# vivek87799/lightweight-human-pose-estimation.pytorch

Measured on AMD Instinct MI355X. Metric: frames/sec end-to-end (net+grouping) at 368px, higher is better.
Workload: dtype f32; 1 GPU; batch=1 per GPU, 368x656 frames, 1 refinement stage(s), fp32 convs / f32+f64 post, resident normalised NCHW input -> key-points + pose entries on host; 3 frame batch(es) in flight per GPU (3 engine stream(s), each step a complete pass); global_batch=1, parallelism=dp1 (frames sharded, no data-path collective), 3 stream(s) per GPU

## Files before the change

lightweight-human-pose-estimation.pytorch_amd/csrc/capi.cpp:

```cpp
#include <algorithm>
#include <cmath>
#include <cstdio>
#include <cstdlib>
#include <cstring>
#include <map>
#include <mutex>
#include <string>
#include <vector>

#include "lwp_internal.h"
#include "lwp_owners.h"

using namespace lwp;

struct lwp_context {
    int device = 0;
    Stream stream, post_own;
    hipStream_t post_stream = nullptr;
    int dtype = LWP_F32;
    Graph g;
    Tuning tune;
    std::vector<std::string> variants;
    bool record_variants = false;
    char variant_buf[kVariantCap] = {0};
// ... 685 lines not shown
    return v;
}

static inline float* buf_at(lwp_context* h, const BufRef& r) {
    const int nb = (int)h->g.bufs.size();
    char* base = (r.buf < nb ? h->bufs[r.buf] : h->tbufs[r.buf - nb]).as<char>();
    return (float*)(base + (size_t)r.coff * (h->dtype != LWP_F32 ? 2 : 4));
}
static inline int buf_level(const lwp_context* h, int buf) {
    const int nb = (int)h->g.bufs.size();
    return buf < 0 ? 0 : buf < nb ? h->g.bufs[buf].level : h->tp.bufs[buf - nb].level;
}

static int enqueue_layer(lwp_context* h, const Layer& l, const float* d_in, int N, int H, int W, float* const* d_outs_nchw,
                         const Layer* fold = nullptr, bool* folded = nullptr) {
    const bool h16 = h->dtype != LWP_F32;
    const int f16 = h->dtype == LWP_F16;
    const float* wts = h->blob(l.w_off);
    const float* bias = h->blob(l.b_off);
    int dh, dw;
    level_dims(H, W, buf_level(h, l.dst.buf), &dh, &dw);
    float* dst = buf_at(h, l.dst);
    char* vb = h->record_variants ? h->variant_buf : nullptr;
    if (vb) vb[0] = 0;
    if (l.kind == L_STEM) {
        StemParams p{d_in, wts, bias, dst, N, H, W, dh, dw, f16, h->d_zeros.as<float>()};
        p.tune = &h->tune; p.variant = vb;
        LAUNCH(h, KC_STEM, h16 ? launch_stem_bf16(p, h->stream) : launch_stem(p, h->stream));
    } else if (l.kind == L_DWPW) {
        int sh, sw;
        level_dims(H, W, buf_level(h, l.src.buf), &sh, &sw);
        DwPwParams p;
        p.in = buf_at(h, l.src); p.in_ld = l.src.ld; p.f16 = f16;
        p.dw_w = wts; p.pw_w = h->blob(l.w2_off); p.pw_b = h->blob(l.b2_off);
        p.out = dst; p.out_ld = l.dst.ld;
        p.res = l.res.buf >= 0 ? buf_at(h, l.res) : nullptr; p.res_ld = l.res.ld;
        p.zeros = h->d_zeros.as<float>();
        p.N = N; p.Hi = sh; p.Wi = sw; p.Ho = dh; p.Wo = dw; p.C = l.cin; p.cout = l.cout;
        p.stride = l.stride; p.dil = l.dil; p.act_dw = l.act; p.act_pw = l.act2;
        p.tune = &h->tune; p.variant = vb;
        LAUNCH(h, KC_PW, h16 ? launch_dwpw_bf16(p, h->stream) : launch_dwpw(p, h->stream));
    } else if (l.kind == L_DW) {
        int sh, sw;
        level_dims(H, W, buf_level(h, l.src.buf), &sh, &sw);
        DwParams p{buf_at(h, l.src), l.src.ld, wts, bias, dst, l.dst.ld, N, sh, sw, dh, dw, l.cin, l.stride, l.dil, l.act};
        p.tune = &h->tune; p.variant = vb;
        LAUNCH(h, KC_DW, launch_dw(p, h->stream));
    } else {
        GemmParams p;
        p.in = buf_at(h, l.src); p.in_ld = l.src.ld; p.f16 = f16;
        p.w = wts; p.bias = bias;
        p.wf = h16 ? nullptr : h->blob(l.w2_off);
        p.out = dst; p.out_ld = l.dst.ld;
        p.res = l.res.buf >= 0 ? buf_at(h, l.res) : nullptr; p.res_ld = l.res.ld;
        p.out_nchw = (l.out_index >= 0 && d_outs_nchw) ? d_outs_nchw[l.out_index] : nullptr;
        p.out_nchw2 = (l.out_index2 >= 0 && d_outs_nchw) ? d_outs_nchw[l.out_index2] : nullptr;
        p.out_split = l.out_split;
        p.zeros = h->d_zeros.as<float>();
        p.N = N; p.H = dh; p.W = dw;
        p.cin_pad = l.cin_pad; p.cout = l.cout; p.cout_pad = l.cout_pad; p.ks = l.ks; p.dil = l.dil; p.act = l.act;
        p.tune = &h->tune; p.variant = vb;
        if (fold) {
            p.w2 = h->blob(fold->w_off); p.bias2 = h->blob(fold->b_off);
            p.out2 = buf_at(h, fold->dst); p.out2_ld = fold->dst.ld; p.act2 = fold->act;
            p.fused2 = folded;
        }
        LAUNCH(h, l.ks == 1 ? KC_PW : KC_C3, h16 ? launch_gemm_bf16(p, h->stream) : launch_gemm(p, h->stream));
    }
    if (vb && h->cur_layer >= 0 && h->cur_layer < (int)h->variants.size()) h->variants[h->cur_layer] = vb;
    return LWP_OK;
}

static bool heads_pair_runs(const lwp_context* h, const Layer& a, const Layer& b, int64_t M) {
    if (a.fuse != LWP_MARK_HEADS_PAIR || h->tune.fuse_heads == 0) return false;
    return h->dtype != LWP_F32 ? heads_bf16_supported(a.cin_pad, a.cout_pad, b.cout_pad) : heads_f32_supported(a.cin_pad, a.cout_pad, b.cout_pad, M, &h->tune);
}

static int enqueue_heads_pair(lwp_context* h, const Layer& a, const Layer& b, int N, int H, int W, float* const* d_outs_nchw) {
    int dh, dw;
    level_dims(H, W, buf_level(h, b.dst.buf), &dh, &dw);
    HeadsParams p;
    p.in = buf_at(h, a.src); p.in_ld = a.src.ld; p.f16 = h->dtype == LWP_F16;
    p.w0 = h->blob(a.w_off); p.b0 = h->blob(a.b_off);
    p.w1 = h->blob(b.w_off); p.b1 = h->blob(b.b_off);
    p.out = buf_at(h, b.dst); p.out_ld = b.dst.ld;
    p.out_nchw = (b.out_index >= 0 && d_outs_nchw) ? d_outs_nchw[b.out_index] : nullptr;
    p.out_nchw2 = (b.out_index2 >= 0 && d_outs_nchw) ? d_outs_nchw[b.out_index2] : nullptr;
    p.out_split = b.out_split;
    p.N = N; p.H = dh; p.W = dw; p.hidden = a.cout_pad; p.cout = b.cout;
    char* vb = h->record_variants ? h->variant_buf : nullptr;
    if (vb) vb[0] = 0;
    p.tune = &h->tune; p.variant = vb;
    LAUNCH(h, KC_PW, h->dtype != LWP_F32 ? launch_heads_bf16(p, h->stream) : launch_heads_f32(p, h->stream));
    if (vb && h->cur_layer >= 0 && h->cur_layer + 1 < (int)h->variants.size()) { h->variants[h->cur_layer] = vb; h->variants[h->cur_layer + 1] = vb; }
    return LWP_OK;
}

static int enqueue_dw_copy(lwp_context* h, const Layer& l, int buf, int N, int H, int W) {
    int sh, sw, dh, dw;
    level_dims(H, W, buf_level(h, l.src.buf), &sh, &sw);
    level_dims(H, W, buf_level(h, buf), &dh, &dw);
    DwParams p{buf_at(h, l.src), l.src.ld, h->blob(l.w_off), h->blob(l.b_off), h->tbufs[buf - (int)h->g.bufs.size()].as<float>(), l.cin,
               N, sh, sw, dh, dw, l.cin, l.stride, l.dil, l.act};
    p.tune = &h->tune;
    LAUNCH(h, KC_DW, launch_dw(p, h->stream));
    return LWP_OK;
}

static int enqueue_forward(lwp_context* h, const std::vector<Layer>& ls, int begin, int end, const float* d_in, int N, int H, int W,
                           float* const* d_outs_nchw, bool retain = false) {
    int fh, fw;
    level_dims(H, W, 3, &fh, &fw);
    const int64_t M3 = (int64_t)N * fh * fw;
    int rc = LWP_OK;
    for (int i = begin; i < end && rc == LWP_OK; ++i) {
        h->cur_layer = i;
        const bool inside = i + 1 < end;
        if (inside && heads_pair_runs(h, ls[i], ls[i + 1], M3)) {
            if (retain) rc = enqueue_layer(h, ls[i], d_in, N, H, W, nullptr);
            if (!rc) rc = enqueue_heads_pair(h, ls[i], ls[i + 1], N, H, W, d_outs_nchw);
            ++i;
            continue;
        }
        if (retain && &ls == &h->tp.layers) {
            if (h->tp.dw_copy[i] >= 0) {
                rc = enqueue_dw_copy(h, ls[i], h->tp.dw_copy[i], N, H, W);
                if (rc) break;
            }
            if (h->tp.nores_copy[i] >= 0) {
                Layer c = ls[i];
                c.res = BufRef();
                c.dst.buf = h->tp.nores_copy[i]; c.dst.coff = 0;
                c.out_index = c.out_index2 = -1;
                rc = enqueue_layer(h, c, d_in, N, H, W, nullptr);
                if (rc) break;
            }
        }
        bool folded = false;
        rc = enqueue_layer(h, ls[i], d_in, N, H, W, d_outs_nchw, inside && ls[i].fuse == LWP_MARK_FOLD_NEXT_1X1 ? &ls[i + 1] : nullptr, &folded);
        if (!rc && folded) {
            if (h->record_variants && (size_t)i + 1 < h->variants.size()) h->variants[i + 1] = h->variants[i];
            ++i;
        }
    }
    h->cur_layer = -1;
    return rc;
}
static int enqueue_network(lwp_context* h, const float* d_in, int N, int H, int W, float* const* d_outs_nchw) {
    return enqueue_forward(h, h->g.layers, 0, (int)h->g.layers.size(), d_in, N, H, W, d_outs_nchw);
}

static int check_frame_shape(lwp_context* h, int N, int H, int W) {
    if (N <= 0 || H <= 0 || W <= 0) return fail(h, LWP_ERR_ARG, "bad frame shape");
    if (H < 8 || W < 8) return fail(h, LWP_ERR_ARG, "frame too small (H, W >= 8)");
    if (!h->weights_loaded) return fail(h, LWP_ERR_STATE, "weights not loaded (call lwp_load_weights first)");
    return LWP_OK;
}

static int stage_input(lwp_context* h, const float* in, int in_mem, size_t bytes, const float** d_in) {
    if (in_mem == LWP_MEM_DEVICE) { *d_in = in; return LWP_OK; }
    HIP_TRY(h, h->d_in.ensure(bytes));
    HIP_TRY(h, hipMemcpyAsync(h->d_in.as<float>(), in, bytes, hipMemcpyHostToDevice, h->stream));
    *d_in = h->d_in.as<float>();
    return LWP_OK;
}

// ... 3495 lines not shown
```

lightweight-human-pose-estimation.pytorch_amd/csrc/lwp_internal.h:

```cpp
#pragma once
#include <hip/hip_runtime.h>
#include <stdint.h>
#include <algorithm>
#include <cstdio>
#include <string>
#include <vector>

#include "../../include/lwpose.h"

namespace lwp {

struct ParamSpec {
    std::string key;
    int64_t shape[4];
    int ndim;
    int role;
};
std::vector<ParamSpec> param_table(int nref, int C, int NH, int NP);

enum LayerKind { L_STEM = 0, L_DW = 1, L_GEMM = 2, L_DWPW = 3 };
enum Act { ACT_NONE = 0, ACT_RELU = 1, ACT_ELU = 2 };
enum KClass { KC_STEM = 0, KC_DW = 1, KC_PW = 2, KC_C3 = 3, KC_POST = 4, KC_OTHER = 5, KC_COUNT = 6 };

struct BufRef {
// ... 11 lines not shown
    int kind = L_GEMM;
    std::string name;
    std::string conv_key;
    std::string bn_key;
    bool has_bias = false;
    int cin = 0, cout = 0, ks = 1, stride = 1, dil = 1, act = ACT_NONE;
    BufRef src, dst, res;
    int out_index = -1;
    int out_index2 = -1, out_split = 0;
    std::vector<WBlock> blocks;
    int64_t macs_per_pixel = 0;
    int fuse = LWP_MARK_NONE;
    size_t w_off = 0, b_off = 0;
    int cin_pad = 0, cout_pad = 0;
    std::string conv2_key, bn2_key;
    int act2 = ACT_NONE;
    size_t w2_off = 0, b2_off = 0;
};

struct BufSpec {
    int level;
    int channels;
    bool has_pad = false;
};

struct Graph {
    int nref, C, NH, NP;
    std::vector<BufSpec> bufs;
    std::vector<Layer> layers;
    size_t blob_floats = 0;
    int cat_buf = -1;
    int cat_channels = 0;
    int dtype = LWP_F32;
};
Graph build_graph(int nref, int C, int NH, int NP, bool fuse_dwpw, int dtype, bool merge_heads = true);

struct TrainPlan {
    std::vector<Layer> layers;
    std::vector<BufSpec> bufs;
    std::vector<int> cats;
    int cpm_conv = -1;
    int cpm_in = -1;
    int cut = -1;
    std::vector<int> dw_copy, nores_copy;
    enum { GRAD_ALWAYS = 0, GRAD_NEVER = 1, GRAD_ON_DEMAND = 2 };
    std::vector<char> grad_mode;
};
TrainPlan build_train_plan(const Graph& g, int scope = LWP_TRAIN_STAGES);
uint16_t f32_to_f16_rne(float f);
uint16_t f32_to_bf16_rne(float f);

struct HostTensor {
    const void* ptr;
    int64_t shape[4];
    int ndim;
};
std::string pack_weights(const Graph& g, const std::vector<std::string>& names,
                         const std::vector<HostTensor>& tensors, std::vector<float>& blob);

struct Tuning {
    int stem_ty = 0, stem_wl = -1, stem_debug = 0;
    int dw_tiled = -1, dw_cc = 0, dw_ph = 0;
    int gemm_wp = -1;
    int gemm_debug = 0;
    bool has_c3 = false, has_pw = false; int c3[3] = {0, 0, 0}, pw[3] = {0, 0, 0};
    int dwpw_bm = 0, dwpw_nw = 0, dwpw_debug = 0, dwpwh_debug = 0;
    int dwpw_pipe = -1;
    int dwpw_tiled_wgs = 0;
    int dwpw_tiled = -1;
    int dwpw_pp_grid = 0;
    int dwpw_pp = -1;
    int heads_rm = 0;
    int gemmh_fold = -1;
    int gemmh_persist = -1, gemmh_ar_off = 0, gemmh_ar_force = 0, gemmh_debug = 0;
    bool has_gemmh_ar = false, has_gemmh = false; int gemmh_ar[4] = {0, 0, 0, 0}, gemmh[4] = {0, 0, 0, 0};
    int upsample_tiled = -1;
    int max_frames_per_pass = 0;
    int peak_tile = -1, pair_form = -1;
    int dwpw_lds_pad_kb = 0;
    int host_fetch_dma = -1;
    int ms_tx = 0;
    int ms_vec = -1;
    int ms_fused = -1;
    int heads_f32_lds = -1;
    int post_nchw = -1;
    int heads_f32_max_m = 0;
    int fuse_dwpw = -1, merge_heads = -1, fuse_heads = -1;
    int pre_batch_vec = -1;
    int post_stream = -1, post_generic = -1;
};
Tuning tuning_from_env();
const Tuning& default_tuning();
constexpr int kVariantCap = 64;
#define LWP_VARIANT(p, ...) do { if ((p).variant) snprintf((p).variant, lwp::kVariantCap, __VA_ARGS__); } while (0)

struct StemParams {
    const float* __restrict__ in;
    const float* __restrict__ w;
    const float* __restrict__ bias;
    float* __restrict__ out;
    int N, H, W, Ho, Wo;
    int f16 = 0;
    const float* zeros = nullptr;
    const Tuning* tune = nullptr; char* variant = nullptr;
};
struct DwParams {
    const float* in; int in_ld;
    const float* w;
    const float* bias;
    float* out; int out_ld;
    int N, Hi, Wi, Ho, Wo, C, stride, dil, act;
    const Tuning* tune = nullptr; char* variant = nullptr;
};
struct GemmParams {
    const float* in; int in_ld;
    int f16 = 0;
    const float* w;
    const float* wf = nullptr;
    const float* bias;
    float* out; int out_ld;
    const float* res; int res_ld;
    float* out_nchw;
    float* out_nchw2 = nullptr;
    int out_split = 0;
    const float* zeros;
    int N, H, W, cin_pad, cout, cout_pad, ks, dil, act;
    int debug = 0;
    const Tuning* tune = nullptr; char* variant = nullptr;
    const void* w2 = nullptr; const float* bias2 = nullptr; void* out2 = nullptr; int out2_ld = 0, act2 = 0;
    bool* fused2 = nullptr;
};
struct DwPwParams {
    const float* in; int in_ld;
    int f16 = 0;
    const float* dw_w;
    const float* pw_w;
    const float* pw_b;
    float* out; int out_ld;
    const float* res; int res_ld;
    const float* zeros;
    int N, Hi, Wi, Ho, Wo, C, cout, stride, dil, act_dw, act_pw;
    int debug = 0;
    const Tuning* tune = nullptr; char* variant = nullptr;
};
bool dwpw_supported(int C, int cout);
hipError_t launch_dwpw(const DwPwParams& p, hipStream_t s);
hipError_t try_dwpw_tiled_f32(const DwPwParams& p, hipStream_t s, bool* used);
hipError_t try_dwpw_tiled_bf16(const DwPwParams& p, hipStream_t s, bool* used);
hipError_t launch_stem_bf16(const StemParams& p, hipStream_t s);
hipError_t launch_dwpw_bf16(const DwPwParams& p, hipStream_t s);
hipError_t launch_gemm_bf16(const GemmParams& p, hipStream_t s);
struct HeadsParams {
    const void* in; int in_ld;
    int f16 = 0;
    const void* w0; const float* b0;
    const void* w1; const float* b1;
    void* out; int out_ld;
    float* out_nchw; float* out_nchw2;
    int out_split, N, H, W, hidden, cout;
    const Tuning* tune = nullptr; char* variant = nullptr;
};
bool heads_bf16_supported(int cin_pad, int hidden, int cout_pad);
hipError_t launch_heads_bf16(const HeadsParams& p, hipStream_t s);
bool heads_f32_supported(int cin_pad, int hidden, int cout_pad, int64_t M, const Tuning* tune = nullptr);
hipError_t launch_heads_f32(const HeadsParams& p, hipStream_t s);
hipError_t launch_nchw_from_nhwc_bf16(const void* src, int src_ld, float* dst, int N, int HW, int C, hipStream_t s, bool f16 = false);
hipError_t launch_stem(const StemParams& p, hipStream_t s);
hipError_t launch_dw(const DwParams& p, hipStream_t s);
hipError_t launch_gemm(const GemmParams& p, hipStream_t s);

struct MapView {
    const float* base;
    int64_t ns, ys, xs, cs;
    int h, w;
};
struct PostCaps { int max_peaks = 2048, max_kpts = 128, max_conn = 4096, max_entries = 256; };

constexpr int kMaxSkelTypes = 64, kMaxSkelLimbs = 320, kMaxEntrySize = 256;
struct Skeleton {
    int K = 18, L = 19, E = 20;
    double min_paf = 0.05;
    std::vector<int> kpt, paf;
    bool is_default = true;
};
Skeleton default_skeleton();

struct PostWorkspace {
    int N = 0;
    PostCaps caps;
    int K = 18, L = 19, E = 20;
    int generic = 0;
    double min_paf = 0.05;
    const int* limbs = nullptr;
    int* peak_count = nullptr;
    uint32_t* peak_key = nullptr;
    float* peak_val = nullptr;
    int* kpt_count = nullptr;
    int* kpt_xy = nullptr;
    float* kpt_score = nullptr;
    int* conn_count = nullptr;
    int* conn_ij = nullptr;
    double* conn_ratio = nullptr;
    unsigned long long* flags = nullptr;
    int* sel_count = nullptr;
    int* seen = nullptr;
    int* sel_ij = nullptr;
    double* sel_r = nullptr;
    float* sel_sa = nullptr;
    float* sel_sb = nullptr;
    double* entries_work = nullptr;
    double* entries = nullptr;
    int* n_entries = nullptr;
    double* kpts_out = nullptr;
    void* result_block = nullptr;
    int tail = 0;
    int* t_n = nullptr;
    unsigned* t_near = nullptr;
    int* t_last = nullptr;
    int* t_ids = nullptr;
    int* t_bbox = nullptr;
    int* t_kp = nullptr;
    double* t_conf = nullptr;
};

struct ResultLayout {
    struct Sec { size_t off, stride; };
    Sec flags, kpts_out, entries, kpt_count, n_entries;
    Sec t_conf, t_bbox, t_kp, t_ids, t_n, t_near, t_last;
    size_t tail_off, bytes;
};
inline ResultLayout result_layout(int N, int K, int E, const PostCaps& c, bool tail) {
    ResultLayout l{};
    size_t q = 0;
    auto sec = [&](ResultLayout::Sec& s, size_t stride) { s.off = q; s.stride = stride; q += (size_t)N * stride; };
    const size_t P = (size_t)c.max_entries;
    sec(l.flags, 4 * 8); sec(l.kpts_out, (size_t)K * c.max_kpts * 4 * 8); sec(l.entries, P * E * 8); sec(l.kpt_count, (size_t)K * 4); sec(l.n_entries, 4);
    l.bytes = q;
    l.tail_off = (q + 15) & ~(size_t)15;
// ... 334 lines not shown
```

lightweight-human-pose-estimation.pytorch_amd/csrc/net_kernels.hip:

```cpp
#include <cstdio>
#include <cstdlib>

#include <type_traits>
#include "lwp_internal.h"

namespace lwp {

typedef float f32x4 __attribute__((ext_vector_type(4)));
typedef float f32x2 __attribute__((ext_vector_type(2)));
typedef float f32x16 __attribute__((ext_vector_type(16)));

__device__ __forceinline__ float elu_negative(float v) {
    const float p = v * (1.f + v * (0.5f + v * (1.f / 6.f + v * (1.f / 24.f + v * (1.f / 120.f + v * (1.f / 720.f + v * (1.f / 5040.f)))))));
    return v > -0.5f ? p : __expf(v) - 1.0f;
}
__device__ __forceinline__ float apply_act(float v, int act) {
    if (act == ACT_RELU) return fmaxf(v, 0.0f);
    if (act == ACT_ELU) return v > 0.0f ? v : elu_negative(v);
    return v;
}

constexpr int ST_TX = 32;
template <bool BF16, int ST_TY, int PY = 1, int DBG = 0, bool WL = false, bool F16 = false>
__global__ void __launch_bounds__(ST_TY * ST_TX) stem_kernel(StemParams p) {
// ... 1400 lines not shown
                }
            }
        }
    }
}

template <int C>
static hipError_t launch_dwpw_pipe_t(const DwPwParams& p, hipStream_t s) {
    const int64_t M = (int64_t)p.N * p.Ho * p.Wo;
    const int ntiles = (int)((M + 31) / 32);
    const size_t lds = (size_t)(2 * 32 * (C + DWPW_F32_APAD) + 10 * C) * sizeof(float);
    static LdsAttrOnce attr;
    hipError_t e = attr.ensure((const void*)dwpw_pipe_kernel<C>, 160 * 1024);
    if (e != hipSuccess) return e;
    int dev = 0, cus = 256;
    if (hipGetDevice(&dev) != hipSuccess || hipDeviceGetAttribute(&cus, hipDeviceAttributeMultiprocessorCount, dev) != hipSuccess || cus <= 0) cus = 256;
    const Tuning& T = p.tune ? *p.tune : default_tuning();
    int grid = cus * (lds <= 80 * 1024 ? 2 : 1);
    if (T.dwpw_pp_grid > 0) grid = T.dwpw_pp_grid;
    if (grid > ntiles) grid = ntiles;
    hipLaunchKernelGGL((dwpw_pipe_kernel<C>), dim3(grid), dim3(1024), lds, s, p, ntiles);
    return hipGetLastError();
}

static hipError_t try_dwpw_pipe(const DwPwParams& p, hipStream_t s, bool* used) {
    *used = false;
    const Tuning& T = p.tune ? *p.tune : default_tuning();
    if (T.dwpw_pipe == 0) return hipSuccess;
    const int64_t M = (int64_t)p.N * p.Ho * p.Wo;
    if (p.cout != 512 || (p.C != 256 && p.C != 512) || p.res || p.act_dw != ACT_RELU || p.act_pw != ACT_RELU) return hipSuccess;
    if ((p.stride != 1 && p.stride != 2) || (p.in_ld & 3) || (p.out_ld & 3) || (((uintptr_t)p.out) & 15) || (((uintptr_t)p.in) & 15)) return hipSuccess;
    if (M >= (1ll << 31) - 64 || (int64_t)p.N * p.Hi * p.Wi * p.in_ld * 4 >= (1ll << 31)) return hipSuccess;
    if (T.dwpw_pipe != 1 && M < 32 * 2048) return hipSuccess;
    if (T.dwpw_pipe != 1 && p.C != 512) return hipSuccess;
    *used = true;
    LWP_VARIANT(p, "dwpw_pipe<%d>", p.C);
    return p.C == 512 ? launch_dwpw_pipe_t<512>(p, s) : launch_dwpw_pipe_t<256>(p, s);
}

bool dwpw_supported(int C, int cout) {
    return C % 32 == 0 && (cout == 64 || cout == 128 || cout == 256 || cout == 512);
}

hipError_t launch_dwpw(const DwPwParams& p_in, hipStream_t s) {
    const DwPwParams& p = p_in;
    {
        bool used = false;
        hipError_t e = try_dwpw_tiled_f32(p, s, &used);
        if (e != hipSuccess || used) return e;
        e = try_dwpw_pipe(p, s, &used);
        if (e != hipSuccess || used) return e;
    }
    const int64_t M = (int64_t)p.N * p.Ho * p.Wo;
    const int nw = p.cout / 32;
    int bm = 16;
    if (M / 32 >= 450) bm = 32;
    if (M / 64 >= 900) bm = 64;
    if (bm == 64 && nw >= 16) bm = 32;
    int nw_wg = nw;
    const Tuning& T = p.tune ? *p.tune : default_tuning();
    if (T.dwpw_bm) bm = T.dwpw_bm;
    if (T.dwpw_nw > 0 && T.dwpw_nw < nw && nw % T.dwpw_nw == 0) nw_wg = T.dwpw_nw;
    if (bm > 64) bm = 64;
    while (bm > 16 && (size_t)bm * (p.C + DWPW_F32_APAD) * sizeof(float) > 150 * 1024) bm >>= 1;
    LWP_VARIANT(p, "dwpw<%d,%d>", bm, nw_wg);
#ifdef LWP_ABLATION
    const int d = T.dwpw_debug;
#define DP_DBG(BM_, NW_, D_) if (bm == BM_ && nw_wg == NW_ && d == D_) return launch_dwpw_t<BM_, NW_, D_>(p, s);
#define DP_DBGS(BM_, NW_) DP_DBG(BM_, NW_, 1) DP_DBG(BM_, NW_, 2) DP_DBG(BM_, NW_, 3) DP_DBG(BM_, NW_, 4) DP_DBG(BM_, NW_, 6) DP_DBG(BM_, NW_, 7) DP_DBG(BM_, NW_, 8)
    DP_DBGS(16, 16) DP_DBGS(16, 8) DP_DBGS(16, 4)
#undef DP_DBGS
#undef DP_DBG
#endif
    const bool relu = p.act_dw == ACT_RELU && p.act_pw == ACT_RELU;
#define DP_CASE(BM_, NW_) if (bm == BM_ && nw_wg == NW_) return relu ? launch_dwpw_t<BM_, NW_, 0, ACT_RELU>(p, s) : launch_dwpw_t<BM_, NW_>(p, s);
    DP_CASE(16, 2) DP_CASE(32, 2) DP_CASE(64, 2)
    DP_CASE(16, 4) DP_CASE(32, 4) DP_CASE(64, 4)
    DP_CASE(16, 8) DP_CASE(32, 8) DP_CASE(64, 8)
    DP_CASE(16, 16) DP_CASE(32, 16) DP_CASE(64, 16)
#undef DP_CASE
    return hipErrorInvalidValue;
}

template <int NW>
__global__ void __launch_bounds__(NW * 64) heads_f32_kernel(HeadsParams p) {
    static_assert(NW == 8, "the reduction maps the 8 waves onto 2 pixel blocks x 4 output tiles");
    extern __shared__ __attribute__((aligned(16))) float hsm[];
    const int tid = threadIdx.x, lane = tid & 63;
    const int wave = __builtin_amdgcn_readfirstlane(tid >> 6);
    const int i16 = lane & 15, q = lane >> 4;
    const int M = p.N * p.H * p.W;
    int bid = blockIdx.x;
    {
        const int nwg = gridDim.x, qq = nwg >> 3, rem = nwg & 7, xcd = bid & 7;
        bid = (xcd < rem ? xcd * (qq + 1) : rem * (qq + 1) + (xcd - rem) * qq) + (bid >> 3);
    }
    const int nheads = p.out_split > 0 ? 2 : 1;
    const int head = nheads == 2 ? (bid & 1) : 0;
    const int ptile = nheads == 2 ? (bid >> 1) : bid;
    int mm[2];
    bool mok[2];
#pragma unroll
    for (int x = 0; x < 2; ++x) { mm[x] = ptile * 32 + x * 16 + i16; mok[x] = mm[x] < M; }
    const float* in = (const float*)p.in;
    const __amdgpu_buffer_rsrc_t xr = __builtin_amdgcn_make_buffer_rsrc((void*)in, 0, (int)((int64_t)M * p.in_ld * 4), 0x00020000);
    const __amdgpu_buffer_rsrc_t w0r = __builtin_amdgcn_make_buffer_rsrc((void*)p.w0, 0, p.hidden * 128 * 4, 0x00020000);
    const __amdgpu_buffer_rsrc_t w1r = __builtin_amdgcn_make_buffer_rsrc((void*)p.w1, 0, 64 * p.hidden * 4, 0x00020000);
    auto ld = [](const __amdgpu_buffer_rsrc_t& r, unsigned voff, unsigned soff) { return __builtin_bit_cast(f32x4, __builtin_amdgcn_raw_buffer_load_b128(r, voff, soff, 0)); };

    const int ntiles = p.hidden / 16 / nheads;
    const int ht0 = head * ntiles;
    const int t_lo = head ? p.out_split / 16 : 0;
    const int nt = (nheads == 2 && !head ? (p.out_split + 15) / 16 : 4) - t_lo;
    const int c_lo = head ? p.out_split : 0, c_hi = (nheads == 2 && !head) ? p.out_split : p.cout;
    const int my = wave < ntiles ? (ntiles - wave + NW - 1) / NW : 0;
    constexpr int HPF = 2;
    f32x4 w0v[HPF][8], w1v[HPF][4], b0v[HPF];
    const __amdgpu_buffer_rsrc_t b0r = __builtin_amdgcn_make_buffer_rsrc((void*)p.b0, 0, p.hidden * 4, 0x00020000);
    const unsigned w0_lane = (unsigned)(i16 * 128 + 32 * q) * 4u, w1_lane = (unsigned)(i16 * p.hidden + 4 * q) * 4u;
    auto request = [&](int k, f32x4* a, f32x4* b, f32x4* bias) {
        const int hl = wave + (k < my ? k : (my > 0 ? my - 1 : 0)) * NW;
        const int htc = ht0 + (hl < ntiles ? hl : 0);
#pragma unroll
        for (int u = 0; u < 8; ++u) a[u] = ld(w0r, w0_lane + 16u * u, (unsigned)htc * (16u * 128u * 4u));
#pragma unroll
        for (int t = 0; t < 4; ++t) {
            const int to = t_lo + (t < nt ? t : nt - 1);
            b[t] = ld(w1r, w1_lane, (unsigned)htc * 64u + (unsigned)(to * 16 * p.hidden) * 4u);
        }
        *bias = ld(b0r, 16u * q, (unsigned)htc * 64u);
    };
    request(0, w0v[0], w1v[0], &b0v[0]);
    f32x4 xf[2][8];
#pragma unroll
    for (int x = 0; x < 2; ++x)
#pragma unroll
        for (int u = 0; u < 8; ++u) xf[x][u] = ld(xr, mok[x] ? (unsigned)((mm[x] * p.in_ld + 32 * q + 4 * u) * 4) : 0x80000000u, 0);

    f32x4 acc2[2][4];
#pragma unroll
    for (int x = 0; x < 2; ++x)
#pragma unroll
        for (int t = 0; t < 4; ++t) acc2[x][t] = f32x4{0.f, 0.f, 0.f, 0.f};
    auto one = [&](int k, auto P_) {
        constexpr int P = decltype(P_)::value;
        request(k + HPF - 1, w0v[(P + HPF - 1) % HPF], w1v[(P + HPF - 1) % HPF], &b0v[(P + HPF - 1) % HPF]);
        __builtin_amdgcn_sched_barrier(0);
        const f32x4 b0 = b0v[P];
        f32x4 acc1[2] = {{0.f, 0.f, 0.f, 0.f}, {0.f, 0.f, 0.f, 0.f}};
#pragma unroll
        for (int u = 0; u < 8; ++u)
#pragma unroll
            for (int c = 0; c < 4; ++c)
#pragma unroll
                for (int x = 0; x < 2; ++x) acc1[x] = __builtin_amdgcn_mfma_f32_16x16x4f32(w0v[P][u][c], xf[x][u][c], acc1[x], 0, 0, 0);
        f32x4 hv[2];
#pragma unroll
        for (int x = 0; x < 2; ++x)
#pragma unroll
            for (int r = 0; r < 4; ++r) hv[x][r] = fmaxf(acc1[x][r] + b0[r], 0.f);
#pragma unroll
        for (int t = 0; t < 4; ++t) {
            if (t >= nt) continue;
#pragma unroll
            for (int r = 0; r < 4; ++r)
#pragma unroll
                for (int x = 0; x < 2; ++x) acc2[x][t] = __builtin_amdgcn_mfma_f32_16x16x4f32(w1v[P][t][r], hv[x][r], acc2[x][t], 0, 0, 0);
        }
    };
    int k = 0;
    for (; k + HPF <= my; k += HPF) {
        one(k, std::integral_constant<int, 0>{});
        one(k + 1, std::integral_constant<int, 1>{});
    }
    if (k < my) one(k, std::integral_constant<int, 0>{});

#pragma unroll
    for (int x = 0; x < 2; ++x)
#pragma unroll
        for (int t = 0; t < 4; ++t) *(f32x4*)(hsm + (((wave * 2 + x) * 4 + t) * 64 + lane) * 4) = acc2[x][t];
    __syncthreads();
    const int x = wave >> 2, t = wave & 3;
    if (t >= nt) return;
    f32x4 v = *(const f32x4*)(hsm + (((0 * 2 + x) * 4 + t) * 64 + lane) * 4);
#pragma unroll
    for (int w = 1; w < NW; ++w) v += *(const f32x4*)(hsm + (((w * 2 + x) * 4 + t) * 64 + lane) * 4);
    const int n = 16 * (t_lo + t) + 4 * q;
    const int m = x ? mm[1] : mm[0];
    if (!(x ? mok[1] : mok[0]) || n >= c_hi || n + 3 < c_lo) return;
    v += *(const f32x4*)(p.b1 + n);
    float* out = (float*)p.out;
    if (((p.out_ld & 3) == 0) && ((((uintptr_t)out) & 15) == 0) && n >= c_lo && n + 3 < c_hi) *(f32x4*)(out + (int64_t)m * p.out_ld + n) = v;
    else {
#pragma unroll
        for (int r = 0; r < 4; ++r) if (n + r >= c_lo && n + r < c_hi) out[(int64_t)m * p.out_ld + n + r] = v[r];
    }
    if (p.out_nchw || p.out_nchw2) {
        const int HW = p.H * p.W;
        const int img = m / HW, pix = m - img * HW;
        const int c0 = p.out_split > 0 ? p.out_split : p.cout;
#pragma unroll
        for (int r = 0; r < 4; ++r) {
            const int ch = n + r;
            if (ch < c_lo || ch >= c_hi) continue;
            if (ch < c0) { if (p.out_nchw) p.out_nchw[((int64_t)img * c0 + ch) * HW + pix] = v[r]; }
            else if (p.out_nchw2) p.out_nchw2[((int64_t)img * (p.cout - c0) + (ch - c0)) * HW + pix] = v[r];
        }
    }
}

constexpr int HL_HC = 32, HL_LD0 = 128 + 8, HL_LD1 = HL_HC + 8;
template <int PT>
__global__ void __launch_bounds__(256) heads_f32_lds_kernel(HeadsParams p) {
    extern __shared__ __attribute__((aligned(16))) float hl_sm[];
    float* W0s = hl_sm;
    float* W1s = W0s + 2 * HL_HC * HL_LD0;
    float* B0s = W1s + 2 * 64 * HL_LD1;
    const int tid = threadIdx.x, lane = tid & 63;
    const int wave = __builtin_amdgcn_readfirstlane(tid >> 6);
    const int i16 = lane & 15, q = lane >> 4;
    const int M = p.N * p.H * p.W;
    int bid = blockIdx.x;
    {
        const int nwg = gridDim.x, qq = nwg >> 3, rem = nwg & 7, xcd = bid & 7;
        bid = (xcd < rem ? xcd * (qq + 1) : rem * (qq + 1) + (xcd - rem) * qq) + (bid >> 3);
    }
    int mr[PT];
    bool mok[PT];
#pragma unroll
    for (int i = 0; i < PT; ++i) { mr[i] = bid * (64 * PT) + (wave * PT + i) * 16 + i16; mok[i] = mr[i] < M; }
    const int nch = p.hidden / HL_HC;
    const float* in = (const float*)p.in;
    const __amdgpu_buffer_rsrc_t xr = __builtin_amdgcn_make_buffer_rsrc((void*)in, 0, (int)((int64_t)M * p.in_ld * 4), 0x00020000);
    const __amdgpu_buffer_rsrc_t w0r = __builtin_amdgcn_make_buffer_rsrc((void*)p.w0, 0, p.hidden * 128 * 4, 0x00020000);
    const __amdgpu_buffer_rsrc_t w1r = __builtin_amdgcn_make_buffer_rsrc((void*)p.w1, 0, 64 * p.hidden * 4, 0x00020000);
    auto ld = [](const __amdgpu_buffer_rsrc_t& r, unsigned voff, unsigned soff) { return __builtin_bit_cast(f32x4, __builtin_amdgcn_raw_buffer_load_b128(r, voff, soff, 0)); };
    f32x4 st0[4], st1[2];
    auto request = [&](int c) {
#pragma unroll
        for (int u = 0; u < 4; ++u) {
            const int ch = tid + u * 256, row = ch >> 5, col = (ch & 31) * 4;
            st0[u] = ld(w0r, (unsigned)(row * 128 + col) * 4u, (unsigned)c * (HL_HC * 128 * 4));
        }
#pragma unroll
        for (int u = 0; u < 2; ++u) {
            const int ch = tid + u * 256, row = ch >> 3, col = (ch & 7) * 4;
            st1[u] = ld(w1r, (unsigned)(row * p.hidden + col) * 4u, (unsigned)c * (HL_HC * 4));
        }
    };
    auto land = [&](int buf) {
#pragma unroll
        for (int u = 0; u < 4; ++u) {
            const int ch = tid + u * 256, row = ch >> 5, col = (ch & 31) * 4;
            *(f32x4*)(W0s + (buf * HL_HC + row) * HL_LD0 + col) = st0[u];
        }
#pragma unroll
        for (int u = 0; u < 2; ++u) {
            const int ch = tid + u * 256, row = ch >> 3, col = (ch & 7) * 4;
// ... 23 lines not shown
        request(c + 1 < nch ? c + 1 : c);
        __builtin_amdgcn_sched_barrier(0);
#pragma unroll
        for (int j = 0; j < HL_HC / 16; ++j) {
            const float* w0 = W0s + (buf * HL_HC + j * 16 + i16) * HL_LD0 + 4 * q;
            f32x4 wv[8];
#pragma unroll
            for (int u = 0; u < 8; ++u) wv[u] = *(const f32x4*)(w0 + 16 * u);
            const f32x4 b0 = *(const f32x4*)(B0s + c * HL_HC + j * 16 + 4 * q);
            const int ht16 = (c * HL_HC + j * 16);
            const bool first_half = ht16 < hsplit;
            const int t_lo = first_half ? 0 : t_first_hi, t_hi = first_half ? t_last_lo : 4;
            f32x4 w1v[4];
#pragma unroll
            for (int t = 0; t < 4; ++t) w1v[t] = *(const f32x4*)(W1s + (buf * 64 + t * 16 + i16) * HL_LD1 + j * 16 + 4 * q);
            __builtin_amdgcn_sched_barrier(0);
            f32x4 acc1[PT];
#pragma unroll
            for (int i = 0; i < PT; ++i) acc1[i] = f32x4{0.f, 0.f, 0.f, 0.f};
#pragma unroll
            for (int u = 0; u < 8; ++u)
#pragma unroll
                for (int cc = 0; cc < 4; ++cc)
#pragma unroll
                    for (int i = 0; i < PT; ++i) acc1[i] = __builtin_amdgcn_mfma_f32_16x16x4f32(wv[u][cc], xf[i][u][cc], acc1[i], 0, 0, 0);
            f32x4 hv[PT];
#pragma unroll
            for (int i = 0; i < PT; ++i)
#pragma unroll
                for (int r = 0; r < 4; ++r) hv[i][r] = fmaxf(acc1[i][r] + b0[r], 0.f);
#pragma unroll
            for (int t = 0; t < 4; ++t) {
                if (t < t_lo || t >= t_hi) continue;
#pragma unroll
                for (int r = 0; r < 4; ++r)
#pragma unroll
                    for (int i = 0; i < PT; ++i) acc2[i][t] = __builtin_amdgcn_mfma_f32_16x16x4f32(w1v[t][r], hv[i][r], acc2[i][t], 0, 0, 0);
            }
        }
        if (c + 1 < nch) land(buf ^ 1);
        __syncthreads();
    }

    float* out = (float*)p.out;
    const int HW = p.H * p.W;
    const int c0 = p.out_split > 0 ? p.out_split : p.cout;
    const bool out_vec = ((p.out_ld & 3) == 0) && ((((uintptr_t)out) & 15) == 0);
#pragma unroll
    for (int i = 0; i < PT; ++i) {
        if (!mok[i]) continue;
        const int m = mr[i];
        const int img = m / HW, pix = m - img * HW;
#pragma unroll
        for (int t = 0; t < 4; ++t) {
            const int n = 16 * t + 4 * q;
            if (n >= p.cout) continue;
            f32x4 v = acc2[i][t];
            v += *(const f32x4*)(p.b1 + n);
            if (out_vec && n + 3 < p.cout) *(f32x4*)(out + (int64_t)m * p.out_ld + n) = v;
            else {
#pragma unroll
                for (int r = 0; r < 4; ++r) if (n + r < p.cout) out[(int64_t)m * p.out_ld + n + r] = v[r];
            }
            if (p.out_nchw || p.out_nchw2) {
#pragma unroll
                for (int r = 0; r < 4; ++r) {
                    const int ch = n + r;
                    if (ch >= p.cout) continue;
                    if (ch < c0) { if (p.out_nchw) p.out_nchw[((int64_t)img * c0 + ch) * HW + pix] = v[r]; }
                    else if (p.out_nchw2) p.out_nchw2[((int64_t)img * (p.cout - c0) + (ch - c0)) * HW + pix] = v[r];
                }
            }
        }
    }
}

bool heads_f32_supported(int cin_pad, int hidden, int cout_pad, int64_t M, const Tuning* tune) {
    const int64_t max_m = (tune && tune->heads_f32_max_m > 0) ? tune->heads_f32_max_m : 4096;
    if (!(cin_pad == 128 && hidden % 16 == 0 && hidden >= 128 && hidden <= 4096 && cout_pad == 64)) return false;
    if (M <= max_m) return true;
    return hidden % HL_HC == 0 && !(tune && tune->heads_f32_lds == 0);
}

hipError_t launch_heads_f32(const HeadsParams& p, hipStream_t s) {
    constexpr int NW = 8;
    const int64_t M = (int64_t)p.N * p.H * p.W;
    if (M * p.in_ld * 4 >= (1ll << 31) || (p.in_ld & 3)) return hipErrorInvalidValue;
    const int64_t max_m = (p.tune && p.tune->heads_f32_max_m > 0) ? p.tune->heads_f32_max_m : 4096;
    if (M > max_m) {
        constexpr int PT = 2;
        if (M >= (1ll << 31) - 64 * PT) return hipErrorInvalidValue;
        const size_t lds2 = (size_t)(2 * HL_HC * HL_LD0 + 2 * 64 * HL_LD1 + p.hidden) * sizeof(float);
        static LdsAttrOnce attr;
        hipError_t e = attr.ensure((const void*)heads_f32_lds_kernel<PT>, 96 * 1024);
        if (e != hipSuccess) return e;
        LWP_VARIANT(p, "heads_f32_lds<%d>", PT);
        hipLaunchKernelGGL(heads_f32_lds_kernel<PT>, dim3((unsigned)((M + 64 * PT - 1) / (64 * PT))), dim3(256), lds2, s, p);
        return hipGetLastError();
    }
    const size_t lds = (size_t)NW * 2 * 4 * 64 * 4 * sizeof(float);
    const unsigned nheads = p.out_split > 0 ? 2u : 1u;
    if (p.out_split < 0 || p.out_split >= p.cout || (nheads == 2 && p.hidden % 32)) return hipErrorInvalidValue;
    static LdsAttrOnce attr8;
    hipError_t e = attr8.ensure((const void*)heads_f32_kernel<NW>, 64 * 1024);
    if (e != hipSuccess) return e;
    LWP_VARIANT(p, "heads_f32<%d>", NW);
    hipLaunchKernelGGL(heads_f32_kernel<NW>, dim3((unsigned)((M + 31) / 32) * nheads), dim3(NW * 64), lds, s, p);
    return hipGetLastError();
}

const Tuning& default_tuning() { static const Tuning t; return t; }
Tuning tuning_from_env() {
    Tuning t;
    auto geti = [](const char* name, int* dst) { const char* e = getenv(name); if (e && e[0]) *dst = atoi(e); };
    auto digit = [](const char* name, int* dst) { const char* e = getenv(name); if (e && e[0]) *dst = e[0] - '0'; };
    geti("LWP_STEM_TY", &t.stem_ty); digit("LWP_STEM_WL", &t.stem_wl); geti("LWP_STEM_DEBUG", &t.stem_debug);
    digit("LWP_DW_TILED", &t.dw_tiled); geti("LWP_DW_CC", &t.dw_cc); geti("LWP_DW_PH", &t.dw_ph);
    digit("LWP_GEMM_WP", &t.gemm_wp);
    if (const char* e = getenv("LWP_GEMM_C3")) t.has_c3 = sscanf(e, "%d,%d,%d", &t.c3[0], &t.c3[1], &t.c3[2]) == 3;
    if (const char* e = getenv("LWP_GEMM_PW")) t.has_pw = sscanf(e, "%d,%d,%d", &t.pw[0], &t.pw[1], &t.pw[2]) == 3;
    geti("LWP_DWPW_BM", &t.dwpw_bm); geti("LWP_DWPW_NW", &t.dwpw_nw); geti("LWP_DWPW_DEBUG", &t.dwpw_debug); geti("LWP_DWPWH_DEBUG", &t.dwpwh_debug);
    digit("LWP_DWPW_PIPE", &t.dwpw_pipe);
    digit("LWP_DWPW_TILED", &t.dwpw_tiled); geti("LWP_DWPW_TILED_WGS", &t.dwpw_tiled_wgs);
    digit("LWP_DWPW_PP", &t.dwpw_pp); geti("LWP_DWPW_PP_GRID", &t.dwpw_pp_grid);
    geti("LWP_HEADS_RM", &t.heads_rm);
    digit("LWP_GEMMH_PERSIST", &t.gemmh_persist); digit("LWP_GEMMH_FOLD", &t.gemmh_fold);
    if (const char* e = getenv("LWP_GEMMH_AR")) {
        if (e[0] == '0' && e[1] == 0) t.gemmh_ar_off = 1;
        else t.has_gemmh_ar = sscanf(e, "%d,%d,%d,%d", &t.gemmh_ar[0], &t.gemmh_ar[1], &t.gemmh_ar[2], &t.gemmh_ar[3]) == 4;
    }
    if (const char* e = getenv("LWP_GEMMH_AR_FORCE")) t.gemmh_ar_force = e[0] == '1';
    geti("LWP_GEMMH_DEBUG", &t.gemmh_debug); geti("LWP_GEMM_DEBUG", &t.gemm_debug);
    if (const char* e = getenv("LWP_GEMMH")) t.has_gemmh = sscanf(e, "%d,%d,%d,%d", &t.gemmh[0], &t.gemmh[1], &t.gemmh[2], &t.gemmh[3]) == 4;
    digit("LWP_UPSAMPLE_TILED", &t.upsample_tiled);
    digit("LWP_PEAK_TILE", &t.peak_tile); digit("LWP_PAIR_FORM", &t.pair_form); digit("LWP_POST_NCHW", &t.post_nchw); digit("LWP_HEADS_F32_LDS", &t.heads_f32_lds); digit("LWP_MS_FUSED", &t.ms_fused); digit("LWP_MS_VEC", &t.ms_vec); geti("LWP_MS_TX", &t.ms_tx); digit("LWP_HOST_FETCH_DMA", &t.host_fetch_dma); geti("LWP_DWPW_LDS_PAD", &t.dwpw_lds_pad_kb);
    geti("LWP_HEADS_F32_MAXM", &t.heads_f32_max_m);
    geti("LWP_MAX_FRAMES_PER_PASS", &t.max_frames_per_pass);
    digit("LWP_FUSE_DWPW", &t.fuse_dwpw); digit("LWP_MERGE_HEADS", &t.merge_heads); digit("LWP_FUSE_HEADS", &t.fuse_heads);
    digit("LWP_PRE_BATCH_VEC", &t.pre_batch_vec); digit("LWP_POST_STREAM", &t.post_stream); digit("LWP_POST_GENERIC", &t.post_generic);
    return t;
}

__global__ void __launch_bounds__(256) nchw_from_nhwc_kernel(const float* src, int src_ld, float* dst, int N, int HW, int C) {
    const int64_t total = (int64_t)N * C * HW;
    const int64_t idx = (int64_t)blockIdx.x * blockDim.x + threadIdx.x;
    if (idx >= total) return;
    const int pix = (int)(idx % HW);
    const int64_t t = idx / HW;
    const int c = (int)(t % C);
    const int n = (int)(t / C);
    dst[idx] = src[((int64_t)n * HW + pix) * src_ld + c];
}
hipError_t launch_nchw_from_nhwc(const float* src, int src_ld, float* dst, int N, int HW, int C, hipStream_t s) {
    const int64_t total = (int64_t)N * C * HW;
    hipLaunchKernelGGL(nchw_from_nhwc_kernel, dim3((unsigned)((total + 255) / 256)), dim3(256), 0, s, src, src_ld, dst, N, HW, C);
    return hipGetLastError();
}

}
```

Measured before the change: 2715 frames/s.

## Stage heads input through LDS and read pre-swizzled w0 layout

The fused f32 heads kernel now loads each 32-pixel input tile cooperatively with coalesced 128-bit loads into a padded LDS tile, then reads per-lane fragments from LDS instead of issuing strided global loads. The first-layer weights come from a pre-permuted copy (w2_off blob) laid out so each lane's loads are contiguous. The pipelined loop also skips the useless prefetch on the final iteration. The LDS footprint grows to 96KB and the kernel now requires hidden%32==0 and the reformatted weight blob. Ablation debug variants are added behind a compile flag.

```diff
diff --git a/lightweight-human-pose-estimation.pytorch_amd/csrc/capi.cpp b/lightweight-human-pose-estimation.pytorch_amd/csrc/capi.cpp
--- a/lightweight-human-pose-estimation.pytorch_amd/csrc/capi.cpp
+++ b/lightweight-human-pose-estimation.pytorch_amd/csrc/capi.cpp
@@ -791,6 +791,7 @@
     HeadsParams p;
     p.in = buf_at(h, a.src); p.in_ld = a.src.ld; p.f16 = h->dtype == LWP_F16;
     p.w0 = h->blob(a.w_off); p.b0 = h->blob(a.b_off);
+    if (h->dtype == LWP_F32) p.w0f = h->blob(a.w2_off);
     p.w1 = h->blob(b.w_off); p.b1 = h->blob(b.b_off);
     p.out = buf_at(h, b.dst); p.out_ld = b.dst.ld;
     p.out_nchw = (b.out_index >= 0 && d_outs_nchw) ? d_outs_nchw[b.out_index] : nullptr;
diff --git a/lightweight-human-pose-estimation.pytorch_amd/csrc/lwp_internal.h b/lightweight-human-pose-estimation.pytorch_amd/csrc/lwp_internal.h
--- a/lightweight-human-pose-estimation.pytorch_amd/csrc/lwp_internal.h
+++ b/lightweight-human-pose-estimation.pytorch_amd/csrc/lwp_internal.h
@@ -117,6 +117,7 @@
     int ms_tx = 0;
     int ms_vec = -1;
     int ms_fused = -1;
+    int heads_debug = 0;
     int heads_f32_lds = -1;
     int post_nchw = -1;
     int heads_f32_max_m = 0;
@@ -189,6 +190,7 @@
     const void* in; int in_ld;
     int f16 = 0;
     const void* w0; const float* b0;
+    const float* w0f = nullptr;
     const void* w1; const float* b1;
     void* out; int out_ld;
     float* out_nchw; float* out_nchw2;
diff --git a/lightweight-human-pose-estimation.pytorch_amd/csrc/net_kernels.hip b/lightweight-human-pose-estimation.pytorch_amd/csrc/net_kernels.hip
--- a/lightweight-human-pose-estimation.pytorch_amd/csrc/net_kernels.hip
+++ b/lightweight-human-pose-estimation.pytorch_amd/csrc/net_kernels.hip
@@ -1506,10 +1506,12 @@
     return hipErrorInvalidValue;
 }
 
-template <int NW>
+constexpr int HX_LD = 32 + 4, HX_QS = 32 * HX_LD;
+template <int NW, int DBG = 0>
 __global__ void __launch_bounds__(NW * 64) heads_f32_kernel(HeadsParams p) {
     static_assert(NW == 8, "the reduction maps the 8 waves onto 2 pixel blocks x 4 output tiles");
     extern __shared__ __attribute__((aligned(16))) float hsm[];
+    float* const xs = hsm + NW * 2 * 4 * 64 * 4;
     const int tid = threadIdx.x, lane = tid & 63;
     const int wave = __builtin_amdgcn_readfirstlane(tid >> 6);
     const int i16 = lane & 15, q = lane >> 4;
@@ -1528,7 +1530,7 @@
     for (int x = 0; x < 2; ++x) { mm[x] = ptile * 32 + x * 16 + i16; mok[x] = mm[x] < M; }
     const float* in = (const float*)p.in;
     const __amdgpu_buffer_rsrc_t xr = __builtin_amdgcn_make_buffer_rsrc((void*)in, 0, (int)((int64_t)M * p.in_ld * 4), 0x00020000);
-    const __amdgpu_buffer_rsrc_t w0r = __builtin_amdgcn_make_buffer_rsrc((void*)p.w0, 0, p.hidden * 128 * 4, 0x00020000);
+    const __amdgpu_buffer_rsrc_t w0fr = __builtin_amdgcn_make_buffer_rsrc((void*)p.w0f, 0, p.hidden * 128 * 4, 0x00020000);
     const __amdgpu_buffer_rsrc_t w1r = __builtin_amdgcn_make_buffer_rsrc((void*)p.w1, 0, 64 * p.hidden * 4, 0x00020000);
     auto ld = [](const __amdgpu_buffer_rsrc_t& r, unsigned voff, unsigned soff) { return __builtin_bit_cast(f32x4, __builtin_amdgcn_raw_buffer_load_b128(r, voff, soff, 0)); };
 
@@ -1541,12 +1543,21 @@
     constexpr int HPF = 2;
     f32x4 w0v[HPF][8], w1v[HPF][4], b0v[HPF];
     const __amdgpu_buffer_rsrc_t b0r = __builtin_amdgcn_make_buffer_rsrc((void*)p.b0, 0, p.hidden * 4, 0x00020000);
-    const unsigned w0_lane = (unsigned)(i16 * 128 + 32 * q) * 4u, w1_lane = (unsigned)(i16 * p.hidden + 4 * q) * 4u;
+    const unsigned w0f_lane = (unsigned)q * (unsigned)(p.hidden / 32) * 4096u + 16u * i16, w1_lane = (unsigned)(i16 * p.hidden + 4 * q) * 4u;
+    f32x4 xg[2];
+    if (!(DBG & 1)) {
+#pragma unroll
+        for (int j = 0; j < 2; ++j) {
+            const int idx = tid + j * NW * 64, m = ptile * 32 + (idx >> 5);
+            xg[j] = ld(xr, m < M ? (unsigned)((m * p.in_ld + 4 * (idx & 31)) * 4) : 0x80000000u, 0);
+        }
+    }
     auto request = [&](int k, f32x4* a, f32x4* b, f32x4* bias) {
+        if (DBG & 2) return;
         const int hl = wave + (k < my ? k : (my > 0 ? my - 1 : 0)) * NW;
         const int htc = ht0 + (hl < ntiles ? hl : 0);
 #pragma unroll
-        for (int u = 0; u < 8; ++u) a[u] = ld(w0r, w0_lane + 16u * u, (unsigned)htc * (16u * 128u * 4u));
+        for (int u = 0; u < 8; ++u) a[u] = ld(w0fr, w0f_lane + 512u * u, (unsigned)(htc >> 1) * 4096u + (unsigned)(htc & 1) * 256u);
 #pragma unroll
         for (int t = 0; t < 4; ++t) {
             const int to = t_lo + (t < nt ? t : nt - 1);
@@ -1554,24 +1565,56 @@
         }
         *bias = ld(b0r, 16u * q, (unsigned)htc * 64u);
     };
+    if (DBG & 2) {
+#pragma unroll
+        for (int b = 0; b < HPF; ++b) {
+#pragma unroll
+            for (int u = 0; u < 8; ++u) w0v[b][u] = f32x4{1.f, 1.f, 1.f, 1.f};
+#pragma unroll
+            for (int t = 0; t < 4; ++t) w1v[b][t] = f32x4{1.f, 1.f, 1.f, 1.f};
+            b0v[b] = f32x4{1.f, 1.f, 1.f, 1.f};
+        }
+    }
     request(0, w0v[0], w1v[0], &b0v[0]);
     f32x4 xf[2][8];
+    if (DBG & 1) {
+#pragma unroll
+        for (int x = 0; x < 2; ++x)
+#pragma unroll
+            for (int u = 0; u < 8; ++u) xf[x][u] = f32x4{1.f, 1.f, 1.f, 1.f};
+    } else {
+#pragma unroll
+        for (int j = 0; j < 2; ++j) {
+            const int idx = tid + j * NW * 64, c4 = idx & 31;
+            *(f32x4*)(xs + (c4 >> 3) * HX_QS + (idx >> 5) * HX_LD + 4 * (c4 & 7)) = xg[j];
+        }
+        __syncthreads();
+#pragma unroll
+        for (int x = 0; x < 2; ++x)
+#pragma unroll
+            for (int u = 0; u < 8; ++u) xf[x][u] = *(const f32x4*)(xs + q * HX_QS + (16 * x + i16) * HX_LD + 4 * u);
+    }
+
+    f32x4 acc2[2][4];
 #pragma unroll
     for (int x = 0; x < 2; ++x)
 #pragma unroll
-        for (int u = 0; u < 8; ++u) xf[x][u] = ld(xr, mok[x] ? (unsigned)((mm[x] * p.in_ld + 32 * q + 4 * u) * 4) : 0x80000000u, 0);
-
-    f32x4 acc2[2][4];
-#pragma unroll
-    for (int x = 0; x < 2; ++x)
-#pragma unroll
         for (int t = 0; t < 4; ++t) acc2[x][t] = f32x4{0.f, 0.f, 0.f, 0.f};
-    auto one = [&](int k, auto P_) {
+    auto one = [&](int k, auto P_, auto LAST_) {
         constexpr int P = decltype(P_)::value;
-        request(k + HPF - 1, w0v[(P + HPF - 1) % HPF], w1v[(P + HPF - 1) % HPF], &b0v[(P + HPF - 1) % HPF]);
+        constexpr bool LAST = decltype(LAST_)::value;
+        if constexpr (!LAST) request(k + HPF - 1, w0v[(P + HPF - 1) % HPF], w1v[(P + HPF - 1) % HPF], &b0v[(P + HPF - 1) % HPF]);
         __builtin_amdgcn_sched_barrier(0);
         const f32x4 b0 = b0v[P];
         f32x4 acc1[2] = {{0.f, 0.f, 0.f, 0.f}, {0.f, 0.f, 0.f, 0.f}};
+        if (DBG & 4) {
+#pragma unroll
+            for (int u = 0; u < 8; ++u) asm volatile("" :: "v"(w0v[P][u]), "v"(xf[0][u]), "v"(xf[1][u]));
+#pragma unroll
+            for (int t = 0; t < 4; ++t) asm volatile("" :: "v"(w1v[P][t]));
+            asm volatile("" :: "v"(b0));
+            return;
+        }
 #pragma unroll
         for (int u = 0; u < 8; ++u)
 #pragma unroll
@@ -1593,11 +1636,23 @@
         }
     };
     int k = 0;
-    for (; k + HPF <= my; k += HPF) {
-        one(k, std::integral_constant<int, 0>{});
-        one(k + 1, std::integral_constant<int, 1>{});
-    }
-    if (k < my) one(k, std::integral_constant<int, 0>{});
+    for (; k + HPF < my; k += HPF) {
+        one(k, std::integral_constant<int, 0>{}, std::false_type{});
+        one(k + 1, std::integral_constant<int, 1>{}, std::false_type{});
+    }
+    if (k + HPF == my) {
+        one(k, std::integral_constant<int, 0>{}, std::false_type{});
+        one(k + 1, std::integral_constant<int, 1>{}, std::true_type{});
+    } else if (k < my) one(k, std::integral_constant<int, 0>{}, std::true_type{});
+    if (DBG & 8) {
+        if (p.out_split == 0x7fffffff) {
+#pragma unroll
+            for (int x = 0; x < 2; ++x)
+#pragma unroll
+                for (int t = 0; t < 4; ++t) *(f32x4*)((float*)p.out + ((x * 4 + t) * 64 + lane) * 4) = acc2[x][t];
+        }
+        return;
+    }
 
 #pragma unroll
     for (int x = 0; x < 2; ++x)
@@ -1787,6 +1842,15 @@
     return hidden % HL_HC == 0 && !(tune && tune->heads_f32_lds == 0);
 }
 
+template <int NW, int DBG>
+static hipError_t launch_heads_f32_i(const HeadsParams& p, hipStream_t s, unsigned grid, size_t lds) {
+    static LdsAttrOnce attr;
+    hipError_t e = attr.ensure((const void*)heads_f32_kernel<NW, DBG>, 96 * 1024);
+    if (e != hipSuccess) return e;
+    hipLaunchKernelGGL((heads_f32_kernel<NW, DBG>), dim3(grid), dim3(NW * 64), lds, s, p);
+    return hipGetLastError();
+}
+
 hipError_t launch_heads_f32(const HeadsParams& p, hipStream_t s) {
     constexpr int NW = 8;
     const int64_t M = (int64_t)p.N * p.H * p.W;
@@ -1803,15 +1867,18 @@
         hipLaunchKernelGGL(heads_f32_lds_kernel<PT>, dim3((unsigned)((M + 64 * PT - 1) / (64 * PT))), dim3(256), lds2, s, p);
         return hipGetLastError();
     }
-    const size_t lds = (size_t)NW * 2 * 4 * 64 * 4 * sizeof(float);
+    const size_t lds = ((size_t)NW * 2 * 4 * 64 * 4 + 4 * HX_QS) * sizeof(float);
     const unsigned nheads = p.out_split > 0 ? 2u : 1u;
-    if (p.out_split < 0 || p.out_split >= p.cout || (nheads == 2 && p.hidden % 32)) return hipErrorInvalidValue;
-    static LdsAttrOnce attr8;
-    hipError_t e = attr8.ensure((const void*)heads_f32_kernel<NW>, 64 * 1024);
-    if (e != hipSuccess) return e;
+    if (p.out_split < 0 || p.out_split >= p.cout || p.hidden % 32 || !p.w0f) return hipErrorInvalidValue;
+    const unsigned grid = (unsigned)((M + 31) / 32) * nheads;
     LWP_VARIANT(p, "heads_f32<%d>", NW);
-    hipLaunchKernelGGL(heads_f32_kernel<NW>, dim3((unsigned)((M + 31) / 32) * nheads), dim3(NW * 64), lds, s, p);
-    return hipGetLastError();
+#ifdef LWP_ABLATION
+    const int d = (p.tune ? *p.tune : default_tuning()).heads_debug;
+#define HD_DBG(D_) if (d == D_) return launch_heads_f32_i<NW, D_>(p, s, grid, lds);
+    HD_DBG(1) HD_DBG(2) HD_DBG(4) HD_DBG(8) HD_DBG(7) HD_DBG(15)
+#undef HD_DBG
+#endif
+    return launch_heads_f32_i<NW, 0>(p, s, grid, lds);
 }
 
 const Tuning& default_tuning() { static const Tuning t; return t; }
@@ -1839,7 +1906,7 @@
     if (const char* e = getenv("LWP_GEMMH")) t.has_gemmh = sscanf(e, "%d,%d,%d,%d", &t.gemmh[0], &t.gemmh[1], &t.gemmh[2], &t.gemmh[3]) == 4;
     digit("LWP_UPSAMPLE_TILED", &t.upsample_tiled);
     digit("LWP_PEAK_TILE", &t.peak_tile); digit("LWP_PAIR_FORM", &t.pair_form); digit("LWP_POST_NCHW", &t.post_nchw); digit("LWP_HEADS_F32_LDS", &t.heads_f32_lds); digit("LWP_MS_FUSED", &t.ms_fused); digit("LWP_MS_VEC", &t.ms_vec); geti("LWP_MS_TX", &t.ms_tx); digit("LWP_HOST_FETCH_DMA", &t.host_fetch_dma); geti("LWP_DWPW_LDS_PAD", &t.dwpw_lds_pad_kb);
-    geti("LWP_HEADS_F32_MAXM", &t.heads_f32_max_m);
+    geti("LWP_HEADS_F32_MAXM", &t.heads_f32_max_m); geti("LWP_HEADS_DEBUG", &t.heads_debug);
     geti("LWP_MAX_FRAMES_PER_PASS", &t.max_frames_per_pass);
     digit("LWP_FUSE_DWPW", &t.fuse_dwpw); digit("LWP_MERGE_HEADS", &t.merge_heads); digit("LWP_FUSE_HEADS", &t.fuse_heads);
     digit("LWP_PRE_BATCH_VEC", &t.pre_batch_vec); digit("LWP_POST_STREAM", &t.post_stream); digit("LWP_POST_GENERIC", &t.post_generic);
```

After: 2781 frames/s (median of 6 runs). 1.02x the previous value.
